# valeoai/rainbow-iqn-apex

Measured on NVIDIA H100. Metric: learner grad-steps/sec (batch=512, N=N'=64), higher is better.
Workload: dtype fp16 fwd / bf16 bwd tensor-core products, fp32 accumulate; fp32 elsewhere

## Files before the change

### rainbow_iqn_apex_b200/csrc/gemm_tc.cu

```cuda
#include <cuda.h>
#include <cudaTypedefs.h>
#include <algorithm>
#include <map>
#include <mutex>
#include <tuple>

#include "common.cuh"
#include "gemm.h"
#include "../../include/riqn_b200.h"

namespace riqn {

using bf16 = __nv_bfloat16;

constexpr int TBM = 128, TBK = 64, MMA_K = 16;
constexpr int kConsumerWGs = 2;
constexpr int kEpiWarps = 4 * kConsumerWGs;
constexpr int kTcThreads = 128 * (1 + kConsumerWGs);
constexpr uint32_t kSlabStride = 72, kSlabBytes = 64 * kSlabStride * 4;
constexpr uint32_t kSmemLimit = 232448;

template <int NSPLIT, int BN, int EPI, bool TMAEPI = false>
struct TcCfg {
  static constexpr int kAOps = NSPLIT == 3 ? 2 : 1, kBOps = NSPLIT == 1 ? 1 : 2;
  static constexpr int kOps = kAOps;
  static constexpr uint32_t kABytes = TBM * TBK * 2, kBBytes = BN * TBK * 2;
  static constexpr uint32_t kStageBytes = kAOps * kABytes + kBOps * kBBytes;
  static constexpr uint32_t kEpiF32Bytes = EPI == TC_BIAS_RELU ? 64 * 32 * 4 : 0;
  static constexpr uint32_t kEpiChunkBytes = kEpiF32Bytes + (EPI == TC_EMBED ? 2 : 1) * 64 * 32 * 2;
  static constexpr int kEpiStages = EPI == TC_EMBED ? 2 : 3;
  static constexpr int kEpiBufsMax = EPI == TC_EMBED ? 6 : BN / 32;
  static constexpr int kEpiBufsFit = (kSmemLimit - 1024 - 256 - kEpiStages * kStageBytes) / (kConsumerWGs * kEpiChunkBytes);
  static constexpr int kEpiBufs = kEpiBufsFit > kEpiBufsMax ? kEpiBufsMax : kEpiBufsFit;
  static constexpr uint32_t kEpiBytes = TMAEPI ? kConsumerWGs * kEpiBufs * kEpiChunkBytes : kConsumerWGs * kSlabBytes;
  static_assert(!TMAEPI || (kEpiBufs >= 2 && (EPI == TC_EMBED ? BN == 128
                                                              : BN == 256 && NSPLIT == 1 && (EPI == TC_BIAS_RELU || EPI == TC_STORE))),
                "TMA-store epilogue: 128x256 single-pass TC_BIAS_RELU / TC_STORE or 128x128 TC_EMBED, at least two staging buffers");
  static_assert(TMAEPI || EPI != TC_EMBED, "the embedding has no slab epilogue");
  static constexpr uint32_t kRingBytes = kSmemLimit - 1024  - kEpiBytes - 256 ;
  static constexpr int kStages = kRingBytes / kStageBytes > 6 ? 6 : kRingBytes / kStageBytes;
  static constexpr uint32_t kSmemBytes = kStages * kStageBytes + 1024 + kEpiBytes + 256;
  static_assert(kSmemBytes <= kSmemLimit && kStages >= 2, "exceeds the 227 KB per-CTA shared memory limit");
  static_assert(!TMAEPI || kStages >= kEpiStages, "the staging budget above assumes a ring of kEpiStages");
};

__device__ __forceinline__ uint32_t smem_u32(const void* p) { return (uint32_t)__cvta_generic_to_shared(p); }

__device__ __forceinline__ void mbar_init(uint64_t* bar, uint32_t count) {
  asm volatile("mbarrier.init.shared::cta.b64 [%0], %1;" ::"r"(smem_u32(bar)), "r"(count));
}
__device__ __forceinline__ void mbar_expect_tx(uint64_t* bar, uint32_t bytes) {
  asm volatile("mbarrier.arrive.expect_tx.shared::cta.b64 _, [%0], %1;" ::"r"(smem_u32(bar)), "r"(bytes) : "memory");
}
__device__ __forceinline__ void mbar_arrive(uint64_t* bar) {
  asm volatile("mbarrier.arrive.shared::cta.b64 _, [%0];" ::"r"(smem_u32(bar)) : "memory");
}
__device__ __forceinline__ void mbar_wait(uint64_t* bar, uint32_t parity) {
  asm volatile(
      "{\n"
      ".reg .pred p;\n"
      "WAIT_%=:\n"
      "mbarrier.try_wait.parity.shared::cta.b64 p, [%0], %1;\n"
      "@p bra DONE_%=;\n"
      "bra WAIT_%=;\n"
      "DONE_%=:\n"
      "}\n" ::"r"(smem_u32(bar)),
      "r"(parity)
      : "memory");
}
__device__ __forceinline__ void tma_load_2d(void* dst, const CUtensorMap* map, int c0, int c1, uint64_t* bar) {
  asm volatile(
      "cp.async.bulk.tensor.2d.shared::cluster.global.mbarrier::complete_tx::bytes [%0], [%1, {%2, %3}], [%4];"
      ::"r"(smem_u32(dst)), "l"(reinterpret_cast<uint64_t>(map)), "r"(c0), "r"(c1), "r"(smem_u32(bar))
      : "memory");
}
__device__ __forceinline__ void tma_store_2d(const CUtensorMap* map, uint32_t src, int c0, int c1) {
  asm volatile("cp.async.bulk.tensor.2d.global.shared::cta.bulk_group [%0, {%1, %2}], [%3];" ::"l"(reinterpret_cast<uint64_t>(map)),
               "r"(c0), "r"(c1), "r"(src)
               : "memory");
}
__device__ __forceinline__ void tma_store_commit() { asm volatile("cp.async.bulk.commit_group;" ::: "memory"); }
__device__ __forceinline__ void tma_store_wait_read() { asm volatile("cp.async.bulk.wait_group.read 0;" ::: "memory"); }
template <int N>
__device__ __forceinline__ void tma_store_wait_read_n() { asm volatile("cp.async.bulk.wait_group.read %0;" ::"n"(N) : "memory"); }
__device__ __forceinline__ void tma_store_wait_all() { asm volatile("cp.async.bulk.wait_group 0;" ::: "memory"); }
__device__ __forceinline__ void fence_proxy_async() { asm volatile("fence.proxy.async.shared::cta;" ::: "memory"); }
__device__ __forceinline__ float2 ldg_nc_f2(const float* p) {
  float2 v;
  asm volatile("ld.global.nc.v2.f32 {%0, %1}, [%2];" : "=f"(v.x), "=f"(v.y) : "l"(p));
  return v;
}
__device__ __forceinline__ void wg_bar(int id) { asm volatile("bar.sync %0, 128;" ::"r"(id) : "memory"); }
__device__ __forceinline__ void wgmma_fence() { asm volatile("wgmma.fence.sync.aligned;" ::: "memory"); }
__device__ __forceinline__ void wgmma_commit() { asm volatile("wgmma.commit_group.sync.aligned;" ::: "memory"); }
template <int N>
__device__ __forceinline__ void wgmma_wait() { asm volatile("wgmma.wait_group.sync.aligned %0;" ::"n"(N) : "memory"); }

template <int N>
struct Wgmma;
template <>
struct Wgmma<32> {
  template <int F16, int TA, int TB>
  static __device__ __forceinline__ void mma(float (&d)[16], uint64_t da, uint64_t db, uint32_t acc) {
#define RIQN_WGMMA(TY) \
    asm volatile( \
        "{\n.reg .pred p;\nsetp.ne.b32 p, %18, 0;\n" \
        "wgmma.mma_async.sync.aligned.m64n32k16.f32." TY "." TY " " \
        "{%0, %1, %2, %3, %4, %5, %6, %7, %8, %9, %10, %11, %12, %13, %14, %15}, %16, %17, p, 1, 1, %19, %20;\n}\n" \
        : \
        "+f"(d[0]), "+f"(d[1]), "+f"(d[2]), "+f"(d[3]), "+f"(d[4]), "+f"(d[5]), "+f"(d[6]), "+f"(d[7]), \
        "+f"(d[8]), "+f"(d[9]), "+f"(d[10]), "+f"(d[11]), "+f"(d[12]), "+f"(d[13]), "+f"(d[14]), "+f"(d[15]) \
        : "l"(da), "l"(db), "r"(acc), "n"(TA), "n"(TB))
    if constexpr (F16) RIQN_WGMMA("f16"); else RIQN_WGMMA("bf16");
#undef RIQN_WGMMA
  }
};

template <>
struct Wgmma<64> {
  template <int F16, int TA, int TB>
  static __device__ __forceinline__ void mma(float (&d)[32], uint64_t da, uint64_t db, uint32_t acc) {
#define RIQN_WGMMA(TY) \
    asm volatile( \
        "{\n.reg .pred p;\nsetp.ne.b32 p, %34, 0;\n" \
        "wgmma.mma_async.sync.aligned.m64n64k16.f32." TY "." TY " " \
        "{%0, %1, %2, %3, %4, %5, %6, %7, %8, %9, %10, %11, %12, %13, %14, %15, %16, %17, %18, %19, %20, %21, %22, %23, %24, %25, %26, %27, %28, %29, %30, %31}, %32, %33, p, 1, 1, %35, %36;\n}\n" \
        : \
        "+f"(d[0]), "+f"(d[1]), "+f"(d[2]), "+f"(d[3]), "+f"(d[4]), "+f"(d[5]), "+f"(d[6]), "+f"(d[7]), \
        "+f"(d[8]), "+f"(d[9]), "+f"(d[10]), "+f"(d[11]), "+f"(d[12]), "+f"(d[13]), "+f"(d[14]), "+f"(d[15]), \
        "+f"(d[16]), "+f"(d[17]), "+f"(d[18]), "+f"(d[19]), "+f"(d[20]), "+f"(d[21]), "+f"(d[22]), "+f"(d[23]), \
        "+f"(d[24]), "+f"(d[25]), "+f"(d[26]), "+f"(d[27]), "+f"(d[28]), "+f"(d[29]), "+f"(d[30]), "+f"(d[31]) \
        : "l"(da), "l"(db), "r"(acc), "n"(TA), "n"(TB))
    if constexpr (F16) RIQN_WGMMA("f16"); else RIQN_WGMMA("bf16");
#undef RIQN_WGMMA
  }
};

template <>
struct Wgmma<128> {
  template <int F16, int TA, int TB>
  static __device__ __forceinline__ void mma(float (&d)[64], uint64_t da, uint64_t db, uint32_t acc) {
#define RIQN_WGMMA(TY) \
    asm volatile( \
        "{\n.reg .pred p;\nsetp.ne.b32 p, %66, 0;\n" \
        "wgmma.mma_async.sync.aligned.m64n128k16.f32." TY "." TY " " \
        "{%0, %1, %2, %3, %4, %5, %6, %7, %8, %9, %10, %11, %12, %13, %14, %15, %16, %17, %18, %19, %20, %21, %22, %23, %24, %25, %26, %27, %28, %29, %30, %31, %32, %33, %34, %35, %36, %37, %38, %39, %40, %41, %42, %43, %44, %45, %46, %47, %48, %49, %50, %51, %52, %53, %54, %55, %56, %57, %58, %59, %60, %61, %62, %63}, %64, %65, p, 1, 1, %67, %68;\n}\n" \
        : \
        "+f"(d[0]), "+f"(d[1]), "+f"(d[2]), "+f"(d[3]), "+f"(d[4]), "+f"(d[5]), "+f"(d[6]), "+f"(d[7]), \
        "+f"(d[8]), "+f"(d[9]), "+f"(d[10]), "+f"(d[11]), "+f"(d[12]), "+f"(d[13]), "+f"(d[14]), "+f"(d[15]), \
        "+f"(d[16]), "+f"(d[17]), "+f"(d[18]), "+f"(d[19]), "+f"(d[20]), "+f"(d[21]), "+f"(d[22]), "+f"(d[23]), \
        "+f"(d[24]), "+f"(d[25]), "+f"(d[26]), "+f"(d[27]), "+f"(d[28]), "+f"(d[29]), "+f"(d[30]), "+f"(d[31]), \
        "+f"(d[32]), "+f"(d[33]), "+f"(d[34]), "+f"(d[35]), "+f"(d[36]), "+f"(d[37]), "+f"(d[38]), "+f"(d[39]), \
        "+f"(d[40]), "+f"(d[41]), "+f"(d[42]), "+f"(d[43]), "+f"(d[44]), "+f"(d[45]), "+f"(d[46]), "+f"(d[47]), \
        "+f"(d[48]), "+f"(d[49]), "+f"(d[50]), "+f"(d[51]), "+f"(d[52]), "+f"(d[53]), "+f"(d[54]), "+f"(d[55]), \
        "+f"(d[56]), "+f"(d[57]), "+f"(d[58]), "+f"(d[59]), "+f"(d[60]), "+f"(d[61]), "+f"(d[62]), "+f"(d[63]) \
        : "l"(da), "l"(db), "r"(acc), "n"(TA), "n"(TB))
    if constexpr (F16) RIQN_WGMMA("f16"); else RIQN_WGMMA("bf16");
#undef RIQN_WGMMA
  }
};

template <>
struct Wgmma<256> {
  template <int F16, int TA, int TB>
  static __device__ __forceinline__ void mma(float (&d)[128], uint64_t da, uint64_t db, uint32_t acc) {
#define RIQN_WGMMA(TY) \
    asm volatile( \
        "{\n.reg .pred p;\nsetp.ne.b32 p, %130, 0;\n" \
        "wgmma.mma_async.sync.aligned.m64n256k16.f32." TY "." TY " " \
        "{%0, %1, %2, %3, %4, %5, %6, %7, %8, %9, %10, %11, %12, %13, %14, %15, %16, %17, %18, %19, %20, %21, %22, %23, %24, %25, %26, %27, %28, %29, %30, %31, %32, %33, %34, %35, %36, %37, %38, %39, %40, %41, %42, %43, %44, %45, %46, %47, %48, %49, %50, %51, %52, %53, %54, %55, %56, %57, %58, %59, %60, %61, %62, %63, %64, %65, %66, %67, %68, %69, %70, %71, %72, %73, %74, %75, %76, %77, %78, %79, %80, %81, %82, %83, %84, %85, %86, %87, %88, %89, %90, %91, %92, %93, %94, %95, %96, %97, %98, %99, %100, %101, %102, %103, %104, %105, %106, %107, %108, %109, %110, %111, %112, %113, %114, %115, %116, %117, %118, %119, %120, %121, %122, %123, %124, %125, %126, %127}, %128, %129, p, 1, 1, %131, %132;\n}\n" \
        : \
        "+f"(d[0]), "+f"(d[1]), "+f"(d[2]), "+f"(d[3]), "+f"(d[4]), "+f"(d[5]), "+f"(d[6]), "+f"(d[7]), \
        "+f"(d[8]), "+f"(d[9]), "+f"(d[10]), "+f"(d[11]), "+f"(d[12]), "+f"(d[13]), "+f"(d[14]), "+f"(d[15]), \
        "+f"(d[16]), "+f"(d[17]), "+f"(d[18]), "+f"(d[19]), "+f"(d[20]), "+f"(d[21]), "+f"(d[22]), "+f"(d[23]), \
        "+f"(d[24]), "+f"(d[25]), "+f"(d[26]), "+f"(d[27]), "+f"(d[28]), "+f"(d[29]), "+f"(d[30]), "+f"(d[31]), \
        "+f"(d[32]), "+f"(d[33]), "+f"(d[34]), "+f"(d[35]), "+f"(d[36]), "+f"(d[37]), "+f"(d[38]), "+f"(d[39]), \
        "+f"(d[40]), "+f"(d[41]), "+f"(d[42]), "+f"(d[43]), "+f"(d[44]), "+f"(d[45]), "+f"(d[46]), "+f"(d[47]), \
        "+f"(d[48]), "+f"(d[49]), "+f"(d[50]), "+f"(d[51]), "+f"(d[52]), "+f"(d[53]), "+f"(d[54]), "+f"(d[55]), \
        "+f"(d[56]), "+f"(d[57]), "+f"(d[58]), "+f"(d[59]), "+f"(d[60]), "+f"(d[61]), "+f"(d[62]), "+f"(d[63]), \
        "+f"(d[64]), "+f"(d[65]), "+f"(d[66]), "+f"(d[67]), "+f"(d[68]), "+f"(d[69]), "+f"(d[70]), "+f"(d[71]), \
        "+f"(d[72]), "+f"(d[73]), "+f"(d[74]), "+f"(d[75]), "+f"(d[76]), "+f"(d[77]), "+f"(d[78]), "+f"(d[79]), \
        "+f"(d[80]), "+f"(d[81]), "+f"(d[82]), "+f"(d[83]), "+f"(d[84]), "+f"(d[85]), "+f"(d[86]), "+f"(d[87]), \
        "+f"(d[88]), "+f"(d[89]), "+f"(d[90]), "+f"(d[91]), "+f"(d[92]), "+f"(d[93]), "+f"(d[94]), "+f"(d[95]), \
        "+f"(d[96]), "+f"(d[97]), "+f"(d[98]), "+f"(d[99]), "+f"(d[100]), "+f"(d[101]), "+f"(d[102]), "+f"(d[103]), \
        "+f"(d[104]), "+f"(d[105]), "+f"(d[106]), "+f"(d[107]), "+f"(d[108]), "+f"(d[109]), "+f"(d[110]), "+f"(d[111]), \
        "+f"(d[112]), "+f"(d[113]), "+f"(d[114]), "+f"(d[115]), "+f"(d[116]), "+f"(d[117]), "+f"(d[118]), "+f"(d[119]), \
        "+f"(d[120]), "+f"(d[121]), "+f"(d[122]), "+f"(d[123]), "+f"(d[124]), "+f"(d[125]), "+f"(d[126]), "+f"(d[127]) \
        : "l"(da), "l"(db), "r"(acc), "n"(TA), "n"(TB))
    if constexpr (F16) RIQN_WGMMA("f16"); else RIQN_WGMMA("bf16");
#undef RIQN_WGMMA
  }
};

template <int N>
__device__ __forceinline__ void wgmma_tile(float (&d)[N / 2], uint64_t da, uint64_t db, uint32_t acc, bool f16, int mn) {
  const bool ta = (mn & 1) != 0, tb = (mn & 2) != 0;
  if (f16) {
    if (ta) { if (tb) Wgmma<N>::template mma<1, 1, 1>(d, da, db, acc); else Wgmma<N>::template mma<1, 1, 0>(d, da, db, acc); }
    else    { if (tb) Wgmma<N>::template mma<1, 0, 1>(d, da, db, acc); else Wgmma<N>::template mma<1, 0, 0>(d, da, db, acc); }
  } else {
    if (ta) { if (tb) Wgmma<N>::template mma<0, 1, 1>(d, da, db, acc); else Wgmma<N>::template mma<0, 1, 0>(d, da, db, acc); }
    else    { if (tb) Wgmma<N>::template mma<0, 0, 1>(d, da, db, acc); else Wgmma<N>::template mma<0, 0, 0>(d, da, db, acc); }
  }
}

__device__ __forceinline__ uint64_t gmma_desc_k128(uint32_t saddr) {
  return (uint64_t)((saddr & 0x3FFFF) >> 4) | ((uint64_t)1 << 16) | ((uint64_t)(1024 >> 4) << 32) | ((uint64_t)1 << 62);
}
__device__ __forceinline__ uint64_t gmma_desc_mn128(uint32_t saddr) {
  return (uint64_t)((saddr & 0x3FFFF) >> 4) | ((uint64_t)(8192 >> 4) << 16) | ((uint64_t)(1024 >> 4) << 32) |
         ((uint64_t)1 << 62);
}
__device__ __forceinline__ uint32_t pack16x2(float a, float b, bool f16) {
  if (f16) {
    const __half2 h = __floats2half2_rn(a, b);
    return *reinterpret_cast<const uint32_t*>(&h);
  }
  const __nv_bfloat162 h = __floats2bfloat162_rn(a, b);
  return *reinterpret_cast<const uint32_t*>(&h);
}

constexpr int kStRow = 32;
__device__ __forceinline__ void sts128(uint32_t addr, uint32_t a, uint32_t b, uint32_t c, uint32_t d) {
  asm volatile("st.shared.v4.b32 [%0], {%1, %2, %3, %4};" ::"r"(addr), "r"(a), "r"(b), "r"(c), "r"(d) : "memory");
}
__device__ __forceinline__ uint4 lds128(uint32_t addr) {
  uint4 v;
  asm volatile("ld.shared.v4.b32 {%0, %1, %2, %3}, [%4];" : "=r"(v.x), "=r"(v.y), "=r"(v.z), "=r"(v.w) : "r"(addr) : "memory");
  return v;
}
__device__ __forceinline__ void stage_row(uint32_t st, const uint32_t (&w)[32], int lane) {
  __syncwarp();
  const uint32_t row = st + lane * (kStRow * 4);
#pragma unroll
  for (int j = 0; j < 8; ++j) sts128(row + ((j ^ (lane & 7)) << 4), w[4 * j], w[4 * j + 1], w[4 * j + 2], w[4 * j + 3]);
  __syncwarp();
}
__device__ __forceinline__ uint4 staged_piece(uint32_t st, int r, int piece) {
  return lds128(st + r * (kStRow * 4) + ((piece ^ (r & 7)) << 4));
}
__device__ __forceinline__ void warp_store_rows_f32(uint32_t st, const uint32_t (&w)[32], int lane, float* base, long ld,
                                                    int rows_valid) {
  stage_row(st, w, lane);
  const int sub = lane >> 3, piece = lane & 7;
#pragma unroll
  for (int r0 = 0; r0 < 32; r0 += 4) {
    const int r = r0 + sub;
    if (r < rows_valid) *reinterpret_cast<uint4*>(base + (long)r * ld + piece * 4) = staged_piece(st, r, piece);
  }
}
__device__ __forceinline__ void warp_store_rows_bf16(uint32_t st, const uint32_t (&w)[32], int lane, bf16* hi_base,
                                                     bf16* lo_base, long ld, int rows_valid) {
  stage_row(st, w, lane);
  const int sub = lane >> 3, piece = lane & 7;
  bf16* dstb = piece < 4 ? hi_base : lo_base;
  if (dstb == nullptr) return;
#pragma unroll
  for (int r0 = 0; r0 < 32; r0 += 4) {
    const int r = r0 + sub;
    if (r < rows_valid) *reinterpret_cast<uint4*>(dstb + (long)r * ld + (piece & 3) * 8) = staged_piece(st, r, piece);
  }
}

template <bool NOISY>
__device__ __forceinline__ void warp_accum_rows_f32(uint32_t st, const uint32_t (&w)[32], int lane, float* c, float* out2,
                                                    const float* eps, long ld, int rows_valid, float alpha) {
  stage_row(st, w, lane);
  const int sub = lane >> 3, piece = lane & 7;
#pragma unroll
  for (int r0 = 0; r0 < 32; r0 += 4) {
    const int r = r0 + sub;
    if (r < rows_valid) {
      const uint4 au = staged_piece(st, r, piece);
      const float4 a = make_float4(__uint_as_float(au.x) * alpha, __uint_as_float(au.y) * alpha,
                                   __uint_as_float(au.z) * alpha, __uint_as_float(au.w) * alpha);
      const long off = (long)r * ld + piece * 4;
      float4 o = *reinterpret_cast<const float4*>(c + off);
      o.x += a.x; o.y += a.y; o.z += a.z; o.w += a.w;
      *reinterpret_cast<float4*>(c + off) = o;
      if (NOISY) {
        const float4 e = *reinterpret_cast<const float4*>(eps + off);
        float4 o2 = *reinterpret_cast<const float4*>(out2 + off);
        o2.x += a.x * e.x; o2.y += a.y * e.y; o2.z += a.z * e.z; o2.w += a.w * e.w;
        *reinterpret_cast<float4*>(out2 + off) = o2;
      }
    }
  }
}

__device__ __forceinline__ void store_transposed_pairs(bf16* tb, const uint32_t* w16, int n0, int m, int M, int lane,
                                                       bool row_ok) {
  const uint32_t sel = (lane & 1) ? 0x3276u : 0x5410u;
  uint32_t* tp = reinterpret_cast<uint32_t*>(tb + (long)(n0 + (lane & 1)) * M + (m & ~1));
  const long step = M;
#pragma unroll
  for (int k = 0; k < 16; ++k) {
    const uint32_t mine = w16[k];
    const uint32_t other = __shfl_xor_sync(0xffffffffu, mine, 1);
    if (row_ok) tp[(long)k * step] = __byte_perm(mine, other, sel);
  }
}

template <int TBN>
__device__ __forceinline__ void mma_kblock(float (&d)[TBN / 2], uint32_t sa, uint32_t sb, bool first, bool f16, int mn) {
#pragma unroll
  for (int k = 0; k < TBK / MMA_K; ++k) {
    const uint32_t koff_mn = k * (MMA_K / 8) * 1024;
    const uint32_t koff_k = k * MMA_K * 2;
    const uint64_t da = (mn & 1) ? gmma_desc_mn128(sa + koff_mn) : gmma_desc_k128(sa + koff_k);
    const uint64_t db = (mn & 2) ? gmma_desc_mn128(sb + koff_mn) : gmma_desc_k128(sb + koff_k);
    wgmma_tile<TBN>(d, da, db, (!first || k > 0) ? 1u : 0u, f16, mn);
  }
}

struct alignas(64) TcArgs {
  CUtensorMap mapO[2];
  int M, N, K;
  int m_tiles, n_tiles, k_splits, kb_per_split, kb_total;
  float* C;
  long ldc;
  const float* bias;
  float* out2;
  const float* eps;
  float alpha;
  int vec_acc;
  int ohw;
  int ci_h, ci_w, ci_cin, ci_kh, ci_kw, ci_stride, ci_ow, ci_G, ci_oh;
  const float* feat;
  int batch;
  bf16 *o_hi, *o_lo;
  bf16 *o_hiT, *o_loT;
  int strip_t, strip_G, strip_kc, cv_oh, cv_ow, nx_s, nx_G;
  int mn_major, wg_t, wg_G, wg_kc;
  bf16 *nx_hi, *nx_lo;
  int fmt;
  int grp_mt, a_wrap;
  const float* bias2;
  long part_stride;
};

template <int NSPLIT, int EPI, int BN, int MODE = 0>
__global__ void __launch_bounds__(kTcThreads, 1)
gemm_tc_kernel(const __grid_constant__ CUtensorMap mapA_hi, const __grid_constant__ CUtensorMap mapA_lo,
               const __grid_constant__ CUtensorMap mapB_hi, const __grid_constant__ CUtensorMap mapB_lo,
               const __grid_constant__ TcArgs p) {
  constexpr bool kTmaEpi = (MODE & 8) != 0;
  using Cfg = TcCfg<NSPLIT, BN, EPI, kTmaEpi>;
  constexpr int TBN = BN;
  extern __shared__ uint8_t smem_raw[];
  uint8_t* smem = reinterpret_cast<uint8_t*>((reinterpret_cast<uintptr_t>(smem_raw) + 1023) & ~uintptr_t(1023));
  uint64_t* bars = reinterpret_cast<uint64_t*>(smem + Cfg::kStages * Cfg::kStageBytes + Cfg::kEpiBytes);
  uint64_t* full = bars;
  uint64_t* empty = bars + Cfg::kStages;
  const uint32_t epi_base = (uint32_t)__cvta_generic_to_shared(smem + Cfg::kStages * Cfg::kStageBytes);

  const int warp = threadIdx.x >> 5, lane = threadIdx.x & 31;
  const int total_units = p.m_tiles * p.n_tiles * p.k_splits;

  if (threadIdx.x == 0) {
    asm volatile("prefetch.tensormap [%0];" ::"l"(reinterpret_cast<uint64_t>(&mapA_hi)) : "memory");
    asm volatile("prefetch.tensormap [%0];" ::"l"(reinterpret_cast<uint64_t>(&mapB_hi)) : "memory");
    if (NSPLIT == 3) asm volatile("prefetch.tensormap [%0];" ::"l"(reinterpret_cast<uint64_t>(&mapA_lo)) : "memory");
    if (NSPLIT >= 2) asm volatile("prefetch.tensormap [%0];" ::"l"(reinterpret_cast<uint64_t>(&mapB_lo)) : "memory");
    for (int i = 0; i < Cfg::kStages; ++i) { mbar_init(&full[i], 1); mbar_init(&empty[i], kEpiWarps); }
    asm volatile("fence.mbarrier_init.release.cluster;" ::: "memory");
  }
  __syncthreads();

  if (warp < 4) {
    if constexpr (BN == 256 || EPI == TC_EMBED) asm volatile("setmaxnreg.dec.sync.aligned.u32 40;" ::: "memory");
    if (warp == 0 && lane == 0) {
      int stage = 0;
      uint32_t phase = 0;
      for (int u = blockIdx.x; u < total_units; u += gridDim.x) {
        const int tiles = p.m_tiles * p.n_tiles;
        const int ks = u / tiles, t = u - ks * tiles;
        const int nt = t % p.n_tiles, mt = t / p.n_tiles;
        const int kb0 = ks * p.kb_per_split, kb1 = min(p.kb_total, kb0 + p.kb_per_split);
        for (int kb = kb0; kb < kb1; ++kb) {
          mbar_wait(&empty[stage], phase ^ 1);
          uint8_t* s = smem + stage * Cfg::kStageBytes;
          mbar_expect_tx(&full[stage], Cfg::kStageBytes);
          if constexpr (EPI == TC_CONV_DGRAD) {
            const int dy = kb / p.strip_t, dx = kb - dy * p.strip_t;
            tma_load_2d(s, &mapA_hi, 0, mt * TBM - (dy * p.strip_G + dx), &full[stage]);
#pragma unroll
            for (int i = 0; i < TBN / 64; ++i)
              tma_load_2d(s + Cfg::kABytes + i * 8192, &mapB_hi, kb * p.N + nt * TBN + 64 * i, 0, &full[stage]);
            if (++stage == Cfg::kStages) { stage = 0; phase ^= 1; }
            continue;
          }
          if (NSPLIT == 1 && p.mn_major) {
            const int kk = kb * TBK;
            if (p.mn_major & 1) {
#pragma unroll
              for (int i = 0; i < TBM / 64; ++i) tma_load_2d(s + i * 8192, &mapA_hi, mt * TBM + 64 * i, kk, &full[stage]);
            } else {
              tma_load_2d(s, &mapA_hi, kk, mt * TBM, &full[stage]);
            }
            if (p.mn_major & 2) {
#pragma unroll
              for (int i = 0; i < (TBN >= 64 ? TBN / 64 : 1); ++i) {
                int b_in = nt * TBN + 64 * i, b_row = kk;
                if (p.wg_t) {
                  const int slab = b_in >> 6, sft = slab / p.wg_kc, dy = sft / p.wg_t;
                  b_in = (slab - sft * p.wg_kc) << 6;
                  b_row += dy * p.wg_G + (sft - dy * p.wg_t);
                }
                tma_load_2d(s + Cfg::kOps * Cfg::kABytes + i * 8192, &mapB_hi, b_in, b_row, &full[stage]);
              }
            } else {
              tma_load_2d(s + Cfg::kOps * Cfg::kABytes, &mapB_hi, kk, nt * TBN, &full[stage]);
            }
            if (++stage == Cfg::kStages) { stage = 0; phase ^= 1; }
            continue;
          }
          int a_col = kb * TBK, a_row = mt * TBM;
          const CUtensorMap *mb_hi = &mapB_hi, *mb_lo = &mapB_lo;
          if (EPI == TC_CONV && p.grp_mt && mt >= p.grp_mt) {
            mb_hi = &p.mapO[0];
            mb_lo = &p.mapO[1];
            if (p.a_wrap) a_row = (mt - p.grp_mt) * TBM;
          }
          if (EPI == TC_CONV) {
            const int sft = kb / p.strip_kc, dy = sft / p.strip_t;
            a_col = (kb - sft * p.strip_kc) * TBK;
            a_row += dy * p.strip_G + (sft - dy * p.strip_t);
          }
          tma_load_2d(s, &mapA_hi, a_col, a_row, &full[stage]);
          tma_load_2d(s + Cfg::kOps * Cfg::kABytes, mb_hi, kb * TBK, nt * TBN, &full[stage]);
          if (NSPLIT == 3) tma_load_2d(s + Cfg::kABytes, &mapA_lo, a_col, a_row, &full[stage]);
          if (NSPLIT >= 2)
            tma_load_2d(s + Cfg::kAOps * Cfg::kABytes + Cfg::kBBytes, mb_lo, kb * TBK, nt * TBN, &full[stage]);
          if (++stage == Cfg::kStages) { stage = 0; phase ^= 1; }
        }
      }
    }
    return;
  }

  if constexpr (BN == 256 || EPI == TC_EMBED) asm volatile("setmaxnreg.inc.sync.aligned.u32 232;" ::: "memory");
  const int g = (warp >> 2) - 1;
  const int wq = warp & 3;
  const int band = wq & 1, colhalf = wq >> 1;
  const int quarter = 2 * g + band;
  const uint32_t slab = epi_base + g * kSlabBytes;
  const uint32_t st = slab + wq * (32 * kStRow * 4);
  const bool f16 = (p.fmt & 3) != 0;
  float conv_bias[32];
  if (EPI == TC_CONV) {
#pragma unroll
    for (int j = 0; j < 32; ++j) conv_bias[j] = (32 * colhalf + j < p.N && 32 * colhalf < TBN) ? p.bias[32 * colhalf + j] : 0.f;
  }
  bool conv_grp1 = false;
  int stage = 0;
  uint32_t phase = 0;
  int epi_seq = 0;
  for (int u = blockIdx.x; u < total_units; u += gridDim.x) {
    const int tiles = p.m_tiles * p.n_tiles;
    const int ks = u / tiles, t = u - ks * tiles;
    const int nt = t % p.n_tiles, mt = t / p.n_tiles;
    const int kb0 = ks * p.kb_per_split, kb1 = min(p.kb_total, kb0 + p.kb_per_split);
    if (EPI == TC_CONV && p.grp_mt && (mt >= p.grp_mt) != conv_grp1) {
      conv_grp1 = mt >= p.grp_mt;
      const float* bsrc = conv_grp1 ? p.bias2 : p.bias;
#pragma unroll
      for (int j = 0; j < 32; ++j) conv_bias[j] = (32 * colhalf + j < p.N && 32 * colhalf < TBN) ? bsrc[32 * colhalf + j] : 0.f;
    }
    float acc[TBN / 2];
    float dg_sum[TBN / 2];
    if constexpr (EPI == TC_CONV_DGRAD) {
#pragma unroll
      for (int i = 0; i < TBN / 2; ++i) dg_sum[i] = 0.f;
    }
    float2 e_bias[TBN / 8], e_feat[2][TBN / 8];
    if constexpr (EPI == TC_EMBED) {
      const int m0 = mt * TBM + 64 * g + 16 * wq + (lane >> 2), m1 = m0 + 8;
      const float* f0 = p.feat + (long)((m0 < p.M ? m0 : 0) / p.batch) * p.N;
      const float* f1 = p.feat + (long)((m1 < p.M ? m1 : 0) / p.batch) * p.N;
#pragma unroll
      for (int j = 0; j < TBN / 8; ++j) {
        int n = nt * TBN + 8 * j + 2 * (lane & 3);
        if (n >= p.N) n = 0;
        e_bias[j] = ldg_nc_f2(p.bias + n);
        e_feat[0][j] = ldg_nc_f2(f0 + n);
        e_feat[1][j] = ldg_nc_f2(f1 + n);
      }
    }
    int prev = -1;
    for (int kb = kb0; kb < kb1; ++kb) {
      mbar_wait(&full[stage], phase);
      const uint32_t s0 = smem_u32(smem + stage * Cfg::kStageBytes);
      const uint32_t sa = s0 + g * 8192;
      const uint32_t sb = s0 + Cfg::kOps * Cfg::kABytes;
      wgmma_fence();
      if constexpr (EPI == TC_CONV_DGRAD) {
        mma_kblock<TBN>(acc, sa, sb, true, false, 2);
      } else if constexpr (BN == 256) {
        mma_kblock<TBN>(acc, sa, sb, kb == kb0, (MODE & 4) != 0, MODE & 3);
      } else if (NSPLIT == 1 && p.mn_major) {
#pragma unroll
        for (int k = 0; k < TBK / MMA_K; ++k) {
          const uint32_t koff_mn = k * (MMA_K / 8) * 1024;
          const uint32_t koff_k = k * MMA_K * 2;
          const uint64_t da = (p.mn_major & 1) ? gmma_desc_mn128(sa + koff_mn) : gmma_desc_k128(sa + koff_k);
          const uint64_t db = (p.mn_major & 2) ? gmma_desc_mn128(sb + koff_mn) : gmma_desc_k128(sb + koff_k);
          wgmma_tile<TBN>(acc, da, db, (kb > kb0 || k > 0) ? 1u : 0u, f16, p.mn_major);
        }
      } else {
#pragma unroll
        for (int k = 0; k < TBK / MMA_K; ++k) {
          const uint32_t koff = k * MMA_K * 2;
          const uint64_t a_hi = gmma_desc_k128(sa + koff), b_hi = gmma_desc_k128(sb + koff);
          wgmma_tile<TBN>(acc, a_hi, b_hi, (kb > kb0 || k > 0) ? 1u : 0u, f16, 0);
          if (NSPLIT >= 2) wgmma_tile<TBN>(acc, a_hi, gmma_desc_k128(sb + Cfg::kBBytes + koff), 1u, false, 0);
          if (NSPLIT == 3) wgmma_tile<TBN>(acc, gmma_desc_k128(sa + Cfg::kABytes + koff), b_hi, 1u, false, 0);
        }
      }
      wgmma_commit();
      wgmma_wait<1>();
      if (prev >= 0) {
        __syncwarp();
        if (lane == 0) mbar_arrive(&empty[prev]);
      }
      prev = stage;
      if (++stage == Cfg::kStages) { stage = 0; phase ^= 1; }
      if constexpr (EPI == TC_CONV_DGRAD) {
        wgmma_wait<0>();
#pragma unroll
        for (int i = 0; i < TBN / 2; ++i) dg_sum[i] += acc[i];
      }
    }
    wgmma_wait<0>();
    __syncwarp();
    if (lane == 0) mbar_arrive(&empty[prev]);
    if constexpr (EPI == TC_CONV_DGRAD) {
#pragma unroll
      for (int i = 0; i < TBN / 2; ++i) acc[i] = dg_sum[i];
    }

    if constexpr (kTmaEpi) {
      constexpr int kChunks = TBN / 32;
      constexpr bool kWhole = Cfg::kEpiBufs == kChunks;
      const int row0 = mt * TBM + 64 * g;
      const int nch = min(kChunks, (p.N - nt * TBN + 31) / 32);
      const bool elected = wq == 0 && lane == 0;
      const uint32_t stg = epi_base + g * (Cfg::kEpiBufs * Cfg::kEpiChunkBytes);
      const int fr = 16 * wq + (lane >> 2);
      if (row0 < p.M) {
#pragma unroll
        for (int h = 0; h < kChunks; ++h) {
          if (h >= nch) break;
          const int buf = kWhole ? h : epi_seq % Cfg::kEpiBufs;
          if (!kWhole || h == 0) {
            if (elected) tma_store_wait_read_n<kWhole ? 0 : Cfg::kEpiBufs - 1>();
            wg_bar(1 + g);
          }
          const uint32_t sf = stg + buf * Cfg::kEpiChunkBytes;
          const uint32_t sh = sf + Cfg::kEpiF32Bytes;
#pragma unroll
          for (int jj = 0; jj < 4; ++jj) {
            const int j = 4 * h + jj;
            if constexpr (EPI == TC_EMBED) {
              const bool x_f16 = (p.fmt & 4) != 0;
#pragma unroll
              for (int hh = 0; hh < 2; ++hh) {
                const int r = fr + 8 * hh;
                const float x0 = e_feat[hh][j].x * fmaxf(acc[4 * j + 2 * hh] + e_bias[j].x, 0.f);
                const float x1 = e_feat[hh][j].y * fmaxf(acc[4 * j + 2 * hh + 1] + e_bias[j].y, 0.f);
                if (p.C != nullptr && row0 + r < p.M)
                  *reinterpret_cast<float2*>(p.C + (long)(row0 + r) * p.N + nt * TBN + 8 * j + 2 * (lane & 3)) = make_float2(x0, x1);
                const uint32_t w0 = pack16x2(x0, x1, x_f16);
                const uint32_t w1 = x_f16 ? pack16x2(x0, x1, false)
                                          : pack16x2(x0 - __uint_as_float(w0 << 16), x1 - __uint_as_float(w0 & 0xffff0000u), false);
                const uint32_t so = sh + r * 64 + ((jj ^ ((r >> 1) & 3)) << 4) + 4 * (lane & 3);
                if (p.o_hi != nullptr) asm volatile("st.shared.b32 [%0], %1;" ::"r"(so), "r"(w0) : "memory");
                if (p.o_lo != nullptr) asm volatile("st.shared.b32 [%0], %1;" ::"r"(so + 64 * 32 * 2), "r"(w1) : "memory");
              }
              continue;
            }
            float b0 = 0.f, b1 = 0.f;
            if (EPI == TC_BIAS_RELU) {
              const int n = nt * TBN + 8 * j + 2 * (lane & 3);
              if (n < p.N) b0 = __ldg(p.bias + n);
              if (n + 1 < p.N) b1 = __ldg(p.bias + n + 1);
            }
#pragma unroll
            for (int hh = 0; hh < 2; ++hh) {
              const int r = fr + 8 * hh;
              float x0 = acc[4 * j + 2 * hh], x1 = acc[4 * j + 2 * hh + 1];
              if (EPI == TC_BIAS_RELU) {
                x0 = fmaxf(x0 + b0, 0.f);
                x1 = fmaxf(x1 + b1, 0.f);
                const uint32_t q = 2 * jj + ((lane & 3) >> 1);
                asm volatile("st.shared.v2.f32 [%0], {%1, %2};" ::"r"(sf + r * 128 + ((q ^ (r & 7)) << 4) + 8 * (lane & 1)),
                             "f"(x0), "f"(x1) : "memory");
              }
              if (EPI == TC_STORE || p.o_hi != nullptr) {
                const __nv_bfloat162 hv = __floats2bfloat162_rn(x0, x1);
                asm volatile("st.shared.b32 [%0], %1;" ::"r"(sh + r * 64 + ((jj ^ ((r >> 1) & 3)) << 4) + 4 * (lane & 3)),
                             "r"(*reinterpret_cast<const uint32_t*>(&hv)) : "memory");
              }
            }
          }
          fence_proxy_async();
          if (!kWhole || h == nch - 1) {
            wg_bar(1 + g);
            if (elected) {
#pragma unroll
              for (int i = kWhole ? 0 : h; i <= h; ++i) {
                const uint32_t si = kWhole ? stg + i * Cfg::kEpiChunkBytes : sf;
                const int c0 = nt * TBN + 32 * i;
                if (EPI == TC_EMBED) {
                  if (p.o_hi != nullptr) tma_store_2d(&p.mapO[0], si, c0, row0);
                  if (p.o_lo != nullptr) tma_store_2d(&p.mapO[1], si + 64 * 32 * 2, c0, row0);
                  continue;
                }
                if (EPI == TC_BIAS_RELU) tma_store_2d(&p.mapO[0], si, c0, row0);
                if (EPI == TC_STORE || p.o_hi != nullptr) tma_store_2d(&p.mapO[1], si + Cfg::kEpiF32Bytes, c0, row0);
              }
              tma_store_commit();
            }
          }
          ++epi_seq;
        }
      }
      continue;
    }

#pragma unroll
    for (int h = 0; h < (TBN + 63) / 64; ++h) {
      if (BN == 256 && nt * TBN + 64 * h >= p.N) break;
      wg_bar(1 + g);
      {
        const uint32_t r0 = slab + ((16 * wq + (lane >> 2)) * kSlabStride + 2 * (lane & 3)) * 4;
#pragma unroll
        for (int j = 0; j < 8; ++j) {
          const int jj = 8 * h + j;
          if (jj * 8 < TBN) {
            asm volatile("st.shared.v2.f32 [%0], {%1, %2};" ::"r"(r0 + j * 32), "f"(acc[4 * jj]), "f"(acc[4 * jj + 1]) : "memory");
            asm volatile("st.shared.v2.f32 [%0], {%1, %2};" ::"r"(r0 + 8 * kSlabStride * 4 + j * 32), "f"(acc[4 * jj + 2]),
                         "f"(acc[4 * jj + 3]) : "memory");
          }
        }
      }
      wg_bar(1 + g);
      const int c = 64 * h + 32 * colhalf;
      uint32_t v[32];
      if (c < TBN) {
        const uint32_t rr = slab + ((32 * band + lane) * kSlabStride + 32 * colhalf) * 4;
#pragma unroll
        for (int j = 0; j < 8; ++j) {
          const uint4 x = lds128(rr + 16 * j);
          v[4 * j] = x.x; v[4 * j + 1] = x.y; v[4 * j + 2] = x.z; v[4 * j + 3] = x.w;
        }
      }
      wg_bar(1 + g);
      if (c >= TBN) continue;
      const int m = mt * TBM + quarter * 32 + lane;
      const int n0 = nt * TBN + c;
      if (m < p.M && n0 < p.N) {
        if (EPI == TC_STORE || EPI == TC_BIAS_RELU) {
          float* crow = p.C + ks * p.part_stride + (long)m * p.ldc + n0;
          if (n0 + 32 <= p.N && (EPI == TC_STORE || (p.M & 1) == 0)) {
          } else if (n0 + 32 <= p.N) {
#pragma unroll
            for (int j = 0; j < 32; j += 4) {
              float4 o = make_float4(__uint_as_float(v[j]), __uint_as_float(v[j + 1]), __uint_as_float(v[j + 2]),
                                     __uint_as_float(v[j + 3]));
              if (EPI == TC_BIAS_RELU) {
                const float4 b = *reinterpret_cast<const float4*>(p.bias + n0 + j);
                o.x = fmaxf(o.x + b.x, 0.f); o.y = fmaxf(o.y + b.y, 0.f);
                o.z = fmaxf(o.z + b.z, 0.f); o.w = fmaxf(o.w + b.w, 0.f);
              }
              *reinterpret_cast<float4*>(crow + j) = o;
              if (EPI == TC_BIAS_RELU && p.o_hiT) {
                p.o_hiT[(long)(n0 + j) * p.M + m] = __float2bfloat16_rn(o.x);
                p.o_hiT[(long)(n0 + j + 1) * p.M + m] = __float2bfloat16_rn(o.y);
                p.o_hiT[(long)(n0 + j + 2) * p.M + m] = __float2bfloat16_rn(o.z);
                p.o_hiT[(long)(n0 + j + 3) * p.M + m] = __float2bfloat16_rn(o.w);
              }
            }
          } else {
#pragma unroll
            for (int j = 0; j < 32; ++j) {
              if (n0 + j < p.N) {
                float o = __uint_as_float(v[j]);
                if (EPI == TC_BIAS_RELU) o = fmaxf(o + p.bias[n0 + j], 0.f);
                crow[j] = o;
                if (EPI == TC_BIAS_RELU && p.o_hiT) p.o_hiT[(long)(n0 + j) * p.M + m] = __float2bfloat16_rn(o);
              }
            }
          }
        } else if (EPI == TC_BIAS_RELU_NCHW) {
          const int b = m / p.ohw, pp = m - b * p.ohw;
          float* cb = p.C + ((long)b * p.N + n0) * p.ohw + pp;
#pragma unroll
          for (int j = 0; j < 32; ++j)
            if (n0 + j < p.N) cb[(long)j * p.ohw] = fmaxf(__uint_as_float(v[j]) + p.bias[n0 + j], 0.f);
        } else if (EPI == TC_COL2IM || EPI == TC_CONV || EPI == TC_CONV_DGRAD) {
        } else if (!(p.vec_acc && n0 + 32 <= p.N)) {
          float* crow = p.C + (long)m * p.ldc + n0;
#pragma unroll
          for (int j = 0; j < 32; ++j) {
            if (n0 + j < p.N) {
              const float o = __uint_as_float(v[j]) * (EPI == TC_ATOMIC ? p.alpha : 1.f);
              crow[j] += o;
              if (EPI == TC_NOISY_WGRAD) p.out2[(long)m * p.ldc + n0 + j] += o * p.eps[(long)m * p.ldc + n0 + j];
            }
          }
        }
      }
      if (EPI == TC_CONV && n0 < p.N) {
        const int gg = p.strip_G * p.strip_G;
        const int mm = m < p.M ? m : 0;
        const int b = mm / gg, rem = mm - b * gg;
        const int gy = rem / p.strip_G, gx = rem - gy * p.strip_G;
        const bool valid = m < p.M && gy < p.cv_oh && gx < p.cv_ow;
        float x[32];
#pragma unroll
        for (int j = 0; j < 32; ++j) x[j] = n0 + j < p.N ? fmaxf(__uint_as_float(v[j]) + conv_bias[j], 0.f) : 0.f;
        if (p.C != nullptr && valid) {
          const int plane = p.cv_oh * p.cv_ow;
          float* cb = p.C + ((long)b * p.N + n0) * plane + gy * p.cv_ow + gx;
#pragma unroll
          for (int j = 0; j < 32; ++j)
            if (n0 + j < p.N) cb[(long)j * plane] = x[j];
        }
        if (p.nx_hi != nullptr && n0 + 32 <= p.N) {
          long o = -1;
          if (valid) {
            const int sn = p.nx_s, by = gy / sn, bx = gx / sn;
            const long r = ((long)b * p.nx_G + by) * p.nx_G + bx;
            o = r * ((long)sn * sn * p.N) + (long)((gy - by * sn) * sn + (gx - bx * sn)) * p.N + n0;
          }
          uint32_t hw[32];
#pragma unroll
          for (int j = 0; j < 32; j += 2) {
            const uint32_t hwj = pack16x2(x[j], x[j + 1], false);
            hw[j / 2] = hwj;
            hw[16 + j / 2] = pack16x2(x[j] - __uint_as_float(hwj << 16), x[j + 1] - __uint_as_float(hwj & 0xffff0000u), false);
          }
          stage_row(st, hw, lane);
          const int sub = lane >> 3, piece = lane & 7;
          bf16* dstb = piece < 4 ? p.nx_hi : p.nx_lo;
          uint4 pc[8];
          long orow[8];
#pragma unroll
          for (int i = 0; i < 8; ++i) {
            pc[i] = staged_piece(st, 4 * i + sub, piece);
            orow[i] = __shfl_sync(0xffffffffu, o, 4 * i + sub);
          }
#pragma unroll
          for (int i = 0; i < 8; ++i)
            if (orow[i] >= 0 && dstb != nullptr) *reinterpret_cast<uint4*>(dstb + orow[i] + (piece & 3) * 8) = pc[i];
        }
      }
      if (EPI == TC_COL2IM && n0 < p.N) {
        const int khw = p.ci_kh * p.ci_kw;
        const int kcol = n0 + lane;
        int coff = -1;
        if (kcol < p.N) {
          const int c = kcol / khw, r = kcol - c * khw;
          const int kh = r / p.ci_kw, kw = r - kh * p.ci_kw;
          coff = (c * p.ci_h + kh) * p.ci_w + kw;
        }
        bool row_ok = m < p.M;
        const int mm = row_ok ? m : 0;
        const int b = mm / p.ohw, pp = mm - b * p.ohw;
        const int rw = p.ci_G ? p.ci_G : p.ci_ow;
        const int oh = pp / rw, ow = pp - oh * rw;
        if (p.ci_G) row_ok = row_ok && oh < p.ci_oh && ow < p.ci_ow;
        float* base = p.C + ((long)b * p.ci_cin * p.ci_h + oh * p.ci_stride) * p.ci_w + ow * p.ci_stride;
#pragma unroll
        for (int j = 0; j < 32; ++j) {
          const int off = __shfl_sync(0xffffffffu, coff, j);
          if (row_ok && off >= 0)
            asm volatile("red.global.add.f32 [%0], %1;" ::"l"(base + off), "f"(__uint_as_float(v[j])) : "memory");
        }
      }
      if (EPI == TC_CONV_DGRAD && n0 < p.N) {
        const int kcol = n0 + lane, s = p.ci_stride;
        int coff = -1;
        if (kcol < p.N) {
          const int blk = kcol / p.ci_cin, c = kcol - blk * p.ci_cin, iy = blk / s, ix = blk - iy * s;
          coff = (c * p.ci_h + iy) * p.ci_w + ix;
        }
        const bool row_ok = m < p.M;
        const int gg = p.strip_G * p.strip_G, mm = row_ok ? m : 0;
        const int b = mm / gg, rem = mm - b * gg, gy = rem / p.strip_G, gx = rem - gy * p.strip_G;
        float* base = p.C + ((long)b * p.ci_cin * p.ci_h + gy * s) * p.ci_w + gx * s;
#pragma unroll
        for (int j = 0; j < 32; ++j) {
          const int off = __shfl_sync(0xffffffffu, coff, j);
          if (row_ok && off >= 0) base[off] = __uint_as_float(v[j]);
        }
      }
      if ((EPI == TC_STORE || (EPI == TC_BIAS_RELU && (p.M & 1) == 0) ||
           ((EPI == TC_ATOMIC || EPI == TC_NOISY_WGRAD) && p.vec_acc)) && n0 + 32 <= p.N) {
        const int m_base = mt * TBM + quarter * 32;
        const int rows_valid = min(32, p.M - m_base);
        if (rows_valid > 0) {
          if (EPI == TC_STORE) {
            if (p.o_hi != nullptr) {
              uint32_t hw2[32];
#pragma unroll
              for (int j = 0; j < 16; ++j) {
                const __nv_bfloat162 h2 = __floats2bfloat162_rn(__uint_as_float(v[2 * j]), __uint_as_float(v[2 * j + 1]));
                hw2[j] = *reinterpret_cast<const uint32_t*>(&h2);
                hw2[16 + j] = 0u;
              }
              warp_store_rows_bf16(st, hw2, lane, p.o_hi + (long)m_base * p.N + n0, nullptr, p.N, rows_valid);
            } else {
              warp_store_rows_f32(st, v, lane, p.C + ks * p.part_stride + (long)m_base * p.ldc + n0, p.ldc, rows_valid);
            }
          } else if (EPI == TC_ATOMIC) {
            warp_accum_rows_f32<false>(st, v, lane, p.C + (long)m_base * p.ldc + n0, nullptr, nullptr, p.ldc, rows_valid,
                                       p.alpha);
          } else if (EPI == TC_NOISY_WGRAD) {
            const long o0 = (long)m_base * p.ldc + n0;
            warp_accum_rows_f32<true>(st, v, lane, p.C + o0, p.out2 + o0, p.eps + o0, p.ldc, rows_valid, 1.f);
          } else if (EPI == TC_BIAS_RELU) {
            const float* br = p.bias + n0;
            uint32_t hw[16];
#pragma unroll
            for (int j = 0; j < 32; j += 4) {
              const float4 bb = __ldg(reinterpret_cast<const float4*>(br + j));
              const float x0 = fmaxf(__uint_as_float(v[j]) + bb.x, 0.f), x1 = fmaxf(__uint_as_float(v[j + 1]) + bb.y, 0.f);
              const float x2 = fmaxf(__uint_as_float(v[j + 2]) + bb.z, 0.f), x3 = fmaxf(__uint_as_float(v[j + 3]) + bb.w, 0.f);
              const __nv_bfloat162 h01 = __floats2bfloat162_rn(x0, x1), h23 = __floats2bfloat162_rn(x2, x3);
              hw[j / 2] = *reinterpret_cast<const uint32_t*>(&h01);
              hw[j / 2 + 1] = *reinterpret_cast<const uint32_t*>(&h23);
              v[j] = __float_as_uint(x0); v[j + 1] = __float_as_uint(x1);
              v[j + 2] = __float_as_uint(x2); v[j + 3] = __float_as_uint(x3);
            }
            if (p.o_hiT) store_transposed_pairs(p.o_hiT, hw, n0, m, p.M, lane, m < p.M);
            warp_store_rows_f32(st, v, lane, p.C + ks * p.part_stride + (long)m_base * p.ldc + n0, p.ldc, rows_valid);
            if (p.o_hi) {
              uint32_t hw2[32];
#pragma unroll
              for (int j = 0; j < 16; ++j) { hw2[j] = hw[j]; hw2[16 + j] = 0u; }
              warp_store_rows_bf16(st, hw2, lane, p.o_hi + (long)m_base * p.N + n0, nullptr, p.N, rows_valid);
            }
          }
        }
      }
    }
  }
  if (kTmaEpi && lane == 0) tma_store_wait_all();
}

static PFN_cuTensorMapEncodeTiled_v12000 get_encode() {
  static PFN_cuTensorMapEncodeTiled_v12000 fn = nullptr;
  static std::once_flag once;
  std::call_once(once, [] {
    void* p = nullptr;
    cudaDriverEntryPointQueryResult q;
    if (cudaGetDriverEntryPoint("cuTensorMapEncodeTiled", &p, cudaEnableDefault, &q) == cudaSuccess &&
        q == cudaDriverEntryPointSuccess)
      fn = reinterpret_cast<PFN_cuTensorMapEncodeTiled_v12000>(p);
  });
  return fn;
}

static int make_map(CUtensorMap* map, const bf16* base, long rows, long K, int box_rows) {
  auto enc = get_encode();
  if (!enc) return (int)cudaErrorNotSupported;
  cuuint64_t dims[2] = {(cuuint64_t)K, (cuuint64_t)rows};
  cuuint64_t strides[1] = {(cuuint64_t)(K * sizeof(bf16))};
  cuuint32_t box[2] = {(cuuint32_t)TBK, (cuuint32_t)box_rows};
  cuuint32_t estr[2] = {1, 1};
  CUresult r = enc(map, CU_TENSOR_MAP_DATA_TYPE_BFLOAT16, 2, const_cast<bf16*>(base), dims, strides, box, estr,
                   CU_TENSOR_MAP_INTERLEAVE_NONE, CU_TENSOR_MAP_SWIZZLE_128B, CU_TENSOR_MAP_L2_PROMOTION_L2_256B,
                   CU_TENSOR_MAP_FLOAT_OOB_FILL_NONE);
  return r == CUDA_SUCCESS ? 0 : (int)cudaErrorInvalidValue;
}

static int make_store_map(CUtensorMap* map, const bf16* base, long rows, long cols, int box_rows = 32) {
  auto enc = get_encode();
  if (!enc) return (int)cudaErrorNotSupported;
  cuuint64_t dims[2] = {(cuuint64_t)cols, (cuuint64_t)rows};
  cuuint64_t strides[1] = {(cuuint64_t)(cols * sizeof(bf16))};
  cuuint32_t box[2] = {32, (cuuint32_t)box_rows};
  cuuint32_t estr[2] = {1, 1};
  CUresult r = enc(map, CU_TENSOR_MAP_DATA_TYPE_BFLOAT16, 2, const_cast<bf16*>(base), dims, strides, box, estr,
                   CU_TENSOR_MAP_INTERLEAVE_NONE, CU_TENSOR_MAP_SWIZZLE_64B, CU_TENSOR_MAP_L2_PROMOTION_NONE,
                   CU_TENSOR_MAP_FLOAT_OOB_FILL_NONE);
  return r == CUDA_SUCCESS ? 0 : (int)cudaErrorInvalidValue;
}
static int make_store_map_f32(CUtensorMap* map, const float* base, long rows, long cols, long ld) {
  auto enc = get_encode();
  if (!enc) return (int)cudaErrorNotSupported;
  cuuint64_t dims[2] = {(cuuint64_t)cols, (cuuint64_t)rows};
  cuuint64_t strides[1] = {(cuuint64_t)(ld * sizeof(float))};
  cuuint32_t box[2] = {32, 64};
  cuuint32_t estr[2] = {1, 1};
  CUresult r = enc(map, CU_TENSOR_MAP_DATA_TYPE_FLOAT32, 2, const_cast<float*>(base), dims, strides, box, estr,
                   CU_TENSOR_MAP_INTERLEAVE_NONE, CU_TENSOR_MAP_SWIZZLE_128B, CU_TENSOR_MAP_L2_PROMOTION_NONE,
                   CU_TENSOR_MAP_FLOAT_OOB_FILL_NONE);
  return r == CUDA_SUCCESS ? 0 : (int)cudaErrorInvalidValue;
}

template <int NSPLIT, int EPI, int BN, int MODE = 0>
static int launch_tc(const CUtensorMap& a_hi, const CUtensorMap& a_lo, const CUtensorMap& b_hi, const CUtensorMap& b_lo,
                     const TcArgs& p, cudaStream_t s) {
  using Cfg = TcCfg<NSPLIT, BN, EPI, (MODE & 8) != 0>;
  static PerDeviceOnce attr_once;
  const int attr_dev = PerDeviceOnce::device();
  if (!attr_once.done[attr_dev]) {
    RIQN_CUDA(cudaFuncSetAttribute(gemm_tc_kernel<NSPLIT, EPI, BN, MODE>, cudaFuncAttributeMaxDynamicSharedMemorySize,
                                   (int)Cfg::kSmemBytes));
    attr_once.done[attr_dev] = true;
  }
  int sms = attr_once.sms[attr_dev];
  if (!sms) {
    RIQN_CUDA(cudaDeviceGetAttribute(&sms, cudaDevAttrMultiProcessorCount, attr_dev));
    attr_once.sms[attr_dev] = sms;
  }
  const int units = p.m_tiles * p.n_tiles * p.k_splits;
  const int grid = units < sms ? units : sms;
  gemm_tc_kernel<NSPLIT, EPI, BN, MODE><<<grid, kTcThreads, Cfg::kSmemBytes, s>>>(a_hi, a_lo, b_hi, b_lo, p);
  return (int)cudaGetLastError();
}

__global__ void split_k_reduce_kernel(int M, int N, int splits, long stride, long ldp, const float* __restrict__ part,
                                      float* __restrict__ C, long ldc, float alpha, float* __restrict__ out2,
                                      const float* __restrict__ eps) {
  const long i = (long)blockIdx.x * blockDim.x + threadIdx.x;
  if (i >= (long)M * N) return;
  const long m = i / N, n = i - m * N;
  float acc = 0.f;
  for (int k = 0; k < splits; ++k) acc += part[k * stride + m * ldp + n];
  C[m * ldc + n] += alpha * acc;
  if (out2 != nullptr) out2[m * ldc + n] += acc * eps[m * ldc + n];
}

int gemm_bf16_tc(int M, int N, int K, const bf16* A_hi, const bf16* A_lo, const bf16* B_hi, const bf16* B_lo, float* C,
                 long ldc, int epi, const float* bias, float* out2, const float* eps, int split_k, cudaStream_t s,
                 const TcExtra* ex) {
  if (M <= 0 || N <= 0 || K <= 0) return 0;
  if ((K % 8) && !(ex != nullptr && ex->mn_major == 3)) return (int)cudaErrorInvalidValue;
  const bool split3 = A_lo != nullptr && B_lo != nullptr;
  const bool split2 = A_lo == nullptr && B_lo != nullptr;
  const bool narrow_ok = epi == TC_BIAS_RELU_NCHW || epi == TC_CONV || ((epi == TC_ATOMIC || epi == TC_STORE) && !split3 && !split2);
  const bool strip = epi == TC_CONV;
  if (strip && (ex == nullptr || ex->strip_t < 1 || ex->strip_kc < 1 || ex->strip_G < 1 || N > 64 ||
                K != ex->strip_t * ex->strip_t * ex->strip_kc * TBK || (ex->nx_hi && (N % 32))))
    return (int)cudaErrorInvalidValue;
  const long a_k = strip ? (long)ex->strip_kc * TBK : K;
  const bool dgrad = epi == TC_CONV_DGRAD;
  if (dgrad && (ex == nullptr || split3 || split2 || ex->mn_major || ex->strip_t < 1 || ex->strip_G < 1 || K > TBK ||
                N % 64 || split_k > 1 || ex->ci_cin < 1 || ex->ci_stride < 1 || N != ex->ci_stride * ex->ci_stride * ex->ci_cin ||
                ex->ci_h != ex->strip_G * ex->ci_stride || ex->ci_w != ex->ci_h))
// ... 325 lines not shown
```

Before: 290.1.

## Give each consumer warpgroup whole conv tiles, alternating tiles with pair barriers

For the TC_CONV epilogue, each of the two consumer warpgroups now computes a full 128-row tile (two 64-row accumulators) instead of splitting one tile. The two warpgroups take alternating tiles, and named-barrier handoffs order their use of the shared stage ring. This lets one warpgroup's epilogue overlap with the other's MMA main loop, and register reallocation via setmaxnreg is enabled to hold the doubled accumulators. The cost is higher register pressure, a barrier dependency between the warpgroups, and more complex stage/phase bookkeeping.

New measurement: 292.9 (median of 6 runs). Within noise of the previous version (+1.0%).

```diff
diff --git a/rainbow_iqn_apex_b200/csrc/gemm_tc.cu b/rainbow_iqn_apex_b200/csrc/gemm_tc.cu
--- a/rainbow_iqn_apex_b200/csrc/gemm_tc.cu
+++ b/rainbow_iqn_apex_b200/csrc/gemm_tc.cu
@@ -91,6 +91,8 @@
   return v;
 }
 __device__ __forceinline__ void wg_bar(int id) { asm volatile("bar.sync %0, 128;" ::"r"(id) : "memory"); }
+__device__ __forceinline__ void pair_bar_wait(int id) { asm volatile("bar.sync %0, 256;" ::"r"(id) : "memory"); }
+__device__ __forceinline__ void pair_bar_arrive(int id) { asm volatile("bar.arrive %0, 256;" ::"r"(id) : "memory"); }
 __device__ __forceinline__ void wgmma_fence() { asm volatile("wgmma.fence.sync.aligned;" ::: "memory"); }
 __device__ __forceinline__ void wgmma_commit() { asm volatile("wgmma.commit_group.sync.aligned;" ::: "memory"); }
 template <int N>
@@ -362,13 +364,13 @@
     asm volatile("prefetch.tensormap [%0];" ::"l"(reinterpret_cast<uint64_t>(&mapB_hi)) : "memory");
     if (NSPLIT == 3) asm volatile("prefetch.tensormap [%0];" ::"l"(reinterpret_cast<uint64_t>(&mapA_lo)) : "memory");
     if (NSPLIT >= 2) asm volatile("prefetch.tensormap [%0];" ::"l"(reinterpret_cast<uint64_t>(&mapB_lo)) : "memory");
-    for (int i = 0; i < Cfg::kStages; ++i) { mbar_init(&full[i], 1); mbar_init(&empty[i], kEpiWarps); }
+    for (int i = 0; i < Cfg::kStages; ++i) { mbar_init(&full[i], 1); mbar_init(&empty[i], EPI == TC_CONV ? 4 : kEpiWarps); }
     asm volatile("fence.mbarrier_init.release.cluster;" ::: "memory");
   }
   __syncthreads();
 
   if (warp < 4) {
-    if constexpr (BN == 256 || EPI == TC_EMBED) asm volatile("setmaxnreg.dec.sync.aligned.u32 40;" ::: "memory");
+    if constexpr (BN == 256 || EPI == TC_EMBED || EPI == TC_CONV) asm volatile("setmaxnreg.dec.sync.aligned.u32 40;" ::: "memory");
     if (warp == 0 && lane == 0) {
       int stage = 0;
       uint32_t phase = 0;
@@ -439,7 +441,7 @@
     return;
   }
 
-  if constexpr (BN == 256 || EPI == TC_EMBED) asm volatile("setmaxnreg.inc.sync.aligned.u32 232;" ::: "memory");
+  if constexpr (BN == 256 || EPI == TC_EMBED || EPI == TC_CONV) asm volatile("setmaxnreg.inc.sync.aligned.u32 232;" ::: "memory");
   const int g = (warp >> 2) - 1;
   const int wq = warp & 3;
   const int band = wq & 1, colhalf = wq >> 1;
@@ -452,15 +454,22 @@
 #pragma unroll
     for (int j = 0; j < 32; ++j) conv_bias[j] = (32 * colhalf + j < p.N && 32 * colhalf < TBN) ? p.bias[32 * colhalf + j] : 0.f;
   }
+  constexpr bool kWholeTiles = EPI == TC_CONV;
   bool conv_grp1 = false;
   int stage = 0;
   uint32_t phase = 0;
   int epi_seq = 0;
-  for (int u = blockIdx.x; u < total_units; u += gridDim.x) {
+  for (int u = blockIdx.x + (kWholeTiles ? g * gridDim.x : 0); u < total_units; u += (kWholeTiles ? 2 : 1) * gridDim.x) {
     const int tiles = p.m_tiles * p.n_tiles;
     const int ks = u / tiles, t = u - ks * tiles;
     const int nt = t % p.n_tiles, mt = t / p.n_tiles;
     const int kb0 = ks * p.kb_per_split, kb1 = min(p.kb_total, kb0 + p.kb_per_split);
+    if constexpr (kWholeTiles) {
+      const int pos = (u - (int)blockIdx.x) / (int)gridDim.x * p.kb_total;
+      stage = pos % Cfg::kStages;
+      phase = (pos / Cfg::kStages) & 1;
+      if (u >= (int)gridDim.x) pair_bar_wait(3 + g);
+    }
     if (EPI == TC_CONV && p.grp_mt && (mt >= p.grp_mt) != conv_grp1) {
       conv_grp1 = mt >= p.grp_mt;
       const float* bsrc = conv_grp1 ? p.bias2 : p.bias;
@@ -468,6 +477,7 @@
       for (int j = 0; j < 32; ++j) conv_bias[j] = (32 * colhalf + j < p.N && 32 * colhalf < TBN) ? bsrc[32 * colhalf + j] : 0.f;
     }
     float acc[TBN / 2];
+    float acc1[TBN / 2];
     float dg_sum[TBN / 2];
     if constexpr (EPI == TC_CONV_DGRAD) {
 #pragma unroll
@@ -507,6 +517,19 @@
           const uint64_t db = (p.mn_major & 2) ? gmma_desc_mn128(sb + koff_mn) : gmma_desc_k128(sb + koff_k);
           wgmma_tile<TBN>(acc, da, db, (kb > kb0 || k > 0) ? 1u : 0u, f16, p.mn_major);
         }
+      } else if constexpr (kWholeTiles) {
+        const auto half = [&](float (&d)[TBN / 2], uint32_t sr, int k) {
+          const uint32_t koff = k * MMA_K * 2;
+          const uint64_t a_hi = gmma_desc_k128(sr + koff), b_hi = gmma_desc_k128(sb + koff);
+          wgmma_tile<TBN>(d, a_hi, b_hi, (kb > kb0 || k > 0) ? 1u : 0u, f16, 0);
+          if (NSPLIT >= 2) wgmma_tile<TBN>(d, a_hi, gmma_desc_k128(sb + Cfg::kBBytes + koff), 1u, false, 0);
+          if (NSPLIT == 3) wgmma_tile<TBN>(d, gmma_desc_k128(sr + Cfg::kABytes + koff), b_hi, 1u, false, 0);
+        };
+#pragma unroll
+        for (int k = 0; k < TBK / MMA_K; ++k) {
+          half(acc, s0, k);
+          half(acc1, s0 + 8192, k);
+        }
       } else {
 #pragma unroll
         for (int k = 0; k < TBK / MMA_K; ++k) {
@@ -530,6 +553,9 @@
 #pragma unroll
         for (int i = 0; i < TBN / 2; ++i) dg_sum[i] += acc[i];
       }
+    }
+    if constexpr (kWholeTiles) {
+      if (u + (int)gridDim.x < total_units) pair_bar_arrive(3 + (g ^ 1));
     }
     wgmma_wait<0>();
     __syncwarp();
@@ -629,8 +655,12 @@
     }
 
 #pragma unroll
+    for (int rh = 0; rh < (kWholeTiles ? 2 : 1); ++rh)
+#pragma unroll
     for (int h = 0; h < (TBN + 63) / 64; ++h) {
       if (BN == 256 && nt * TBN + 64 * h >= p.N) break;
+      const float (&ah)[TBN / 2] = rh ? acc1 : acc;
+      const int qtr = kWholeTiles ? 2 * rh + band : quarter;
       wg_bar(1 + g);
       {
         const uint32_t r0 = slab + ((16 * wq + (lane >> 2)) * kSlabStride + 2 * (lane & 3)) * 4;
@@ -638,9 +668,9 @@
         for (int j = 0; j < 8; ++j) {
           const int jj = 8 * h + j;
           if (jj * 8 < TBN) {
-            asm volatile("st.shared.v2.f32 [%0], {%1, %2};" ::"r"(r0 + j * 32), "f"(acc[4 * jj]), "f"(acc[4 * jj + 1]) : "memory");
-            asm volatile("st.shared.v2.f32 [%0], {%1, %2};" ::"r"(r0 + 8 * kSlabStride * 4 + j * 32), "f"(acc[4 * jj + 2]),
-                         "f"(acc[4 * jj + 3]) : "memory");
+            asm volatile("st.shared.v2.f32 [%0], {%1, %2};" ::"r"(r0 + j * 32), "f"(ah[4 * jj]), "f"(ah[4 * jj + 1]) : "memory");
+            asm volatile("st.shared.v2.f32 [%0], {%1, %2};" ::"r"(r0 + 8 * kSlabStride * 4 + j * 32), "f"(ah[4 * jj + 2]),
+                         "f"(ah[4 * jj + 3]) : "memory");
           }
         }
       }
@@ -657,7 +687,7 @@
       }
       wg_bar(1 + g);
       if (c >= TBN) continue;
-      const int m = mt * TBM + quarter * 32 + lane;
+      const int m = mt * TBM + qtr * 32 + lane;
       const int n0 = nt * TBN + c;
       if (m < p.M && n0 < p.N) {
         if (EPI == TC_STORE || EPI == TC_BIAS_RELU) {
@@ -798,7 +828,7 @@
       }
       if ((EPI == TC_STORE || (EPI == TC_BIAS_RELU && (p.M & 1) == 0) ||
            ((EPI == TC_ATOMIC || EPI == TC_NOISY_WGRAD) && p.vec_acc)) && n0 + 32 <= p.N) {
-        const int m_base = mt * TBM + quarter * 32;
+        const int m_base = mt * TBM + qtr * 32;
         const int rows_valid = min(32, p.M - m_base);
         if (rows_valid > 0) {
           if (EPI == TC_STORE) {
```
